# oval-group/GNN_branching

Measured on AMD Instinct MI355X. Metric: ReLU branching scores/sec (subproblems x ambiguous-ReLUs/s), higher is better.
Workload: dtype f32 (bf16x3-split 64x64 blocks); 1 GPU; cifar_base_kw, 256 synthetic subproblems per rank x 1 rank(s) = 256, T=2, p=64, shipped cifar_trained_gnn weights; batch_per_rank=256, ranks=1, global_batch=256, parallelism=dp1

## Files before the change

### gnn_branching_amd/_lib.py

```python
import ctypes as C
import os
import subprocess
import sys

CSRC = os.path.join(os.path.dirname(os.path.abspath(__file__)), "csrc")
LIB_PATH = os.environ.get("GNNB_LIB", os.path.join(CSRC, "libgnnb.so"))
SOURCES = ["gnnb.hip", "gnnb_dev.h", "gnnb_k_mlp.h", "gnnb_k_gather.h", "gnnb_k_fusedq.h", "gnnb_k_edges.h", "gnnb_k_misc.h", "gnnb_pack.h", "gnnb_train.h", "gnnb_k_kw.h"]
HIPCC_FLAGS = ["--offload-arch=gfx950", "-O3", "-std=c++17", "-shared", "-fPIC", "-pthread"]

GNNB_CONV, GNNB_LINEAR, GNNB_RELU, GNNB_FLATTEN = 0, 1, 2, 3


class LayerDesc(C.Structure):
    _fields_ = [("kind", C.c_int32), ("c_in", C.c_int32), ("c_out", C.c_int32), ("kh", C.c_int32),
                ("kw", C.c_int32), ("stride", C.c_int32), ("pad", C.c_int32), ("n_in", C.c_int32),
                ("n_out", C.c_int32), ("weight", C.c_void_p), ("bias", C.c_void_p)]


class Batch(C.Structure):
    _fields_ = [("lb", C.POINTER(C.c_void_p)), ("ub", C.POINTER(C.c_void_p)),
                ("dual", C.POINTER(C.c_void_p)), ("primal", C.POINTER(C.c_void_p)),
                ("x_lp", C.c_void_p), ("prop_w", C.c_void_p), ("prop_b", C.c_void_p), ("mask", C.c_void_p),
                ("n_graph", C.c_int32), ("n_relu", C.c_int32), ("n_primal", C.c_int32)]

# ... 20 lines not shown
    ("gnnb_get_option", C.c_int, [C.c_void_p, C.c_char_p, C.POINTER(C.c_int)]),
    ("gnnb_option_count", C.c_int, []),
    ("gnnb_option_name", C.c_char_p, [C.c_int]),
    ("gnnb_babsr", C.c_int, [C.c_void_p, C.POINTER(C.c_void_p), C.POINTER(C.c_void_p), C.c_int, C.c_void_p, C.c_void_p,
                             C.c_int, C.c_void_p, C.c_void_p, C.c_void_p]),
    ("gnnb_kw_workspace_bytes", C.c_size_t, [C.c_void_p, C.c_int]),
    ("gnnb_kw_bounds", C.c_int, [C.c_void_p, C.POINTER(KwBatch), C.c_int, C.POINTER(C.c_void_p), C.POINTER(C.c_void_p), C.POINTER(C.c_void_p),
                                 C.POINTER(C.c_void_p), C.c_void_p, C.c_void_p, C.c_size_t, C.c_void_p]),
    ("gnnb_mu_projection", C.c_int, [C.c_void_p, C.c_int, C.POINTER(C.c_int)]),
    ("gnnb_destroy", C.c_int, [C.c_void_p]),
    ("gnnb_get_weights", C.c_int, [C.c_void_p, C.c_void_p, C.c_size_t]),
    ("gnnb_set_weights", C.c_int, [C.c_void_p, C.c_void_p, C.c_size_t]),
    ("gnnb_online_create", C.c_int, [C.c_void_p, C.c_float, C.c_float]),
    ("gnnb_online_step", C.c_int, [C.c_void_p, C.POINTER(Batch), C.c_int, C.c_void_p, C.c_void_p, C.c_void_p, C.c_void_p,
                                   C.c_int, C.c_void_p]),
    ("gnnb_online_grad", C.c_int, [C.c_void_p, C.c_void_p, C.c_size_t]),
    ("gnnb_last_error", C.c_char_p, []),
    ("gnnb_abi_version", C.c_int, []),
    ("gnnb_build_id", C.c_char_p, []),
    ("gnnb_describe", C.c_int, [C.c_void_p, C.c_char_p, C.c_size_t]),
    ("gnnb_mu_location", C.c_int, [C.c_void_p, C.c_int, C.c_int, C.POINTER(C.c_size_t), C.POINTER(C.c_size_t)]),
    ("gnnb_set_halfpass_limit", C.c_int, [C.c_void_p, C.c_int]),
    ("gnnb_debug_occupy", C.c_int, [C.c_int, C.c_int, C.c_size_t, C.c_double, C.c_void_p]),
    ("gnnb_profile_enable", C.c_int, [C.c_void_p, C.c_int]),
    ("gnnb_profile_classes", C.c_int, []),
    ("gnnb_profile_class_name", C.c_char_p, [C.c_int]),
    ("gnnb_profile_read", C.c_int, [C.c_void_p, C.POINTER(C.c_double), C.POINTER(C.c_int64), C.c_int, C.c_int]),
    ("gnnb_profile_trace", C.c_int, [C.c_void_p, C.POINTER(C.c_int), C.POINTER(C.c_double), C.c_int]),
]


OPTION_ENV = {
    "GNNB_BF3": ("bf3", lambda v: int(v != 0)),
    "GNNB_FUSE": ("fuse", lambda v: int(v != 0)),
    "GNNB_NO_TOP": ("top", lambda v: int(v == 0)),
    "GNNB_NO_GATHER": ("gather", lambda v: int(v == 0)),
    "GNNB_NO_EMBED_FUSE": ("embed_fuse", lambda v: int(v == 0)),
    "GNNB_NO_DENSE_LDS": ("dense_lds", lambda v: int(v == 0)),
    "GNNB_TAIL_MAX_B": ("tail_max_b", lambda v: max(0, min(v, 1 << 30))),
    "GNNB_TOP_SPLIT": ("top_split", lambda v: 4 if v >= 4 else (2 if v >= 2 else 1)),
    "GNNB_TOP_FUSE_UPD": ("top_fuse_upd", lambda v: int(v != 0)),
    "GNNB_CLSPRE_MAX_B": ("clspre_max_b", lambda v: max(0, min(v, 1 << 30))),
}
OPTIONS = tuple(sorted({o for o, _ in OPTION_ENV.values()}))


# ... 99 lines not shown
```

### gnn_branching_amd/csrc/gnnb.hip

```cpp
#include <hip/hip_runtime.h>

#include <cmath>
#include <cstdarg>
#include <cstdio>
#include <cstdlib>
#include <cstring>
#include <string>
#include <vector>
#include <thread>
#include <unistd.h>
#include <sched.h>
#include <atomic>
#include <condition_variable>
#include <functional>
#include <mutex>

#include "../../include/gnnb.h"
#include "gnnb_pack.h"
#include "gnnb_train.h"

using namespace gnnb;

typedef float f32x16 __attribute__((ext_vector_type(16)));
typedef float f32x4 __attribute__((ext_vector_type(4)));
// ... 261 lines not shown
}

extern "C" int gnnb_create(gnnb_t** out, const float* w_blob, size_t n_floats, int T, int p) {
  if (!out || !w_blob) return fail(GNNB_E_INVALID, "gnnb_create: null argument");
  if (p != P) return fail(GNNB_E_INVALID, "gnnb_create: embedding size %d unsupported (kernels are built for p=64)", p);
  if (T < 1 || T > 16) return fail(GNNB_E_INVALID, "gnnb_create: T=%d out of range", T);
  if (n_floats != blob_floats()) return fail(GNNB_E_INVALID, "gnnb_create: weight blob has %zu floats, expected %zu", n_floats, blob_floats());
  int ndev = 0;
  hipError_t e = hipGetDeviceCount(&ndev);
  if (e != hipSuccess || ndev == 0) return fail(GNNB_E_HIP, "gnnb_create: no HIP device (%s)", hipGetErrorString(e));
  gnnb_t* h = new gnnb_handle();
  h->T = T;
  h->p = p;
  HIPCHK(hipGetDevice(&h->device));
  hipDeviceProp_t prop;
  HIPCHK(hipGetDeviceProperties(&prop, h->device));
  h->n_cu = prop.multiProcessorCount > 0 ? prop.multiProcessorCount : 256;
  if (int rc = load_weights(h, w_blob, nullptr)) return rc;
  HIPCHK(hipMalloc((void**)&h->d_zero, 256 * sizeof(float)));
  HIPCHK(hipMemset(h->d_zero, 0, 256 * sizeof(float)));
  HIPCHK(hipMalloc((void**)&h->d_ctl, 8 * 64 * sizeof(int)));
  HIPCHK(hipMemset(h->d_ctl, 0, 8 * 64 * sizeof(int)));
  HIPCHK(hipFuncSetAttribute((const void*)k_pre<false>, hipFuncAttributeMaxDynamicSharedMemorySize, (PackPreFwd::FLOATS + PackPreBwd::FLOATS) * 4));
  HIPCHK(hipFuncSetAttribute((const void*)k_pre<true>, hipFuncAttributeMaxDynamicSharedMemorySize, PackPreBwdL3::FLOATS * 4));
  HIPCHK(hipFuncSetAttribute((const void*)k_pre_inp, hipFuncAttributeMaxDynamicSharedMemorySize, PackPreInp::FLOATS * 4));
  HIPCHK(hipFuncSetAttribute((const void*)k_node_update<8, false>, hipFuncAttributeMaxDynamicSharedMemorySize, (PackUpd::FLOATS + 4096) * 4));
  HIPCHK(hipFuncSetAttribute((const void*)k_node_update<8, true>, hipFuncAttributeMaxDynamicSharedMemorySize, (PackUpd::FLOATS + 4096) * 4));
  HIPCHK(hipFuncSetAttribute((const void*)k_node_update<8, false, true>, hipFuncAttributeMaxDynamicSharedMemorySize, (PackUpd::FLOATS + 4096) * 4));
  HIPCHK(hipFuncSetAttribute((const void*)k_node_update<8, true, true>, hipFuncAttributeMaxDynamicSharedMemorySize, (PackUpd::FLOATS + 4096) * 4));
  HIPCHK(hipFuncSetAttribute((const void*)k_node_update<12, false, false, true>, hipFuncAttributeMaxDynamicSharedMemorySize, (PackUpdL3::FLOATS + 6144) * 4));
  HIPCHK(hipFuncSetAttribute((const void*)k_node_update<12, true, false, true>, hipFuncAttributeMaxDynamicSharedMemorySize, (PackUpdL3::FLOATS + 6144) * 4));
  HIPCHK(hipFuncSetAttribute((const void*)k_node_update<12, false, true, true>, hipFuncAttributeMaxDynamicSharedMemorySize, (PackUpdL3::FLOATS + 6144) * 4));
  HIPCHK(hipFuncSetAttribute((const void*)k_node_update<12, true, true, true>, hipFuncAttributeMaxDynamicSharedMemorySize, (PackUpdL3::FLOATS + 6144) * 4));
  HIPCHK(hipFuncSetAttribute((const void*)k_input_update, hipFuncAttributeMaxDynamicSharedMemorySize, PackUpdInp::FLOATS * 4));
  HIPCHK(hipFuncSetAttribute((const void*)k_score, hipFuncAttributeMaxDynamicSharedMemorySize, PackScore::FLOATS * 4));
  HIPCHK(hipFuncSetAttribute((const void*)k_gather<false>, hipFuncAttributeMaxDynamicSharedMemorySize, 128 * 1024));
  HIPCHK(hipFuncSetAttribute((const void*)k_gather<true>, hipFuncAttributeMaxDynamicSharedMemorySize, 128 * 1024));
  HIPCHK(hipFuncSetAttribute((const void*)k_gather16<false>, hipFuncAttributeMaxDynamicSharedMemorySize, 128 * 1024));
  HIPCHK(hipFuncSetAttribute((const void*)k_gather16<true>, hipFuncAttributeMaxDynamicSharedMemorySize, 128 * 1024));
  HIPCHK(hipFuncSetAttribute((const void*)k_gather16<false, true>, hipFuncAttributeMaxDynamicSharedMemorySize, 128 * 1024));
  HIPCHK(hipFuncSetAttribute((const void*)k_livesum, hipFuncAttributeMaxDynamicSharedMemorySize, 160 * 1024));
  HIPCHK(hipFuncSetAttribute((const void*)k_gather_input_update<true, false>, hipFuncAttributeMaxDynamicSharedMemorySize, 160 * 1024));
  HIPCHK(hipFuncSetAttribute((const void*)k_gather_input_update<true, true>, hipFuncAttributeMaxDynamicSharedMemorySize, 160 * 1024));
  HIPCHK(hipFuncSetAttribute((const void*)k_gather<false, true>, hipFuncAttributeMaxDynamicSharedMemorySize, 128 * 1024));

#define FUSEDQ_ATTR(L, S, P) HIPCHK(hipFuncSetAttribute((const void*)k_gather_update_q<L, S, P>, hipFuncAttributeMaxDynamicSharedMemorySize, 160 * 1024))
  FUSEDQ_ATTR(16, 0, false); FUSEDQ_ATTR(16, 1, false); FUSEDQ_ATTR(16, 2, false); FUSEDQ_ATTR(32, 1, false); FUSEDQ_ATTR(32, 1, true);
// ... 471 lines not shown

extern "C" int gnnb_mu_location(const gnnb_t* h, int B, int k, size_t* offset_bytes, size_t* n_floats) {
  if (!h || !h->bound) return fail(GNNB_E_STATE, "gnnb_mu_location: no network bound");
  if (k < 0 || k >= (int)h->N.size() || B < 1) return fail(GNNB_E_INVALID, "gnnb_mu_location: bad layer/batch");
  WsLayout w = ws_layout(h, B);
  if (offset_bytes) *offset_bytes = w.mu[k] * sizeof(float);
  if (n_floats) *n_floats = (size_t)B * h->N[k] * 64;
  return GNNB_OK;
}

extern "C" int gnnb_mu_projection(const gnnb_t* h, int k, int* linear_id) {
  if (!h || !linear_id) return fail(GNNB_E_INVALID, "gnnb_mu_projection: null argument");
  if (k < 0 || k >= (int)h->N.size()) return fail(GNNB_E_INVALID, "gnnb_mu_projection: bad layer");
  *linear_id = k < MAXL + 2 ? h->last_proj[k] : -1;
  return GNNB_OK;
}

extern "C" int gnnb_set_halfpass_limit(gnnb_t* h, int n) {
  if (!h) return fail(GNNB_E_INVALID, "null handle");
  h->halfpass_limit = n;
  return GNNB_OK;
}

extern "C" int gnnb_debug_occupy(int n_workgroups, int threads, size_t lds_bytes, double ms, void* stream) {
  if (n_workgroups < 1 || n_workgroups > 4096 || threads < 64 || threads > 1024 || lds_bytes > 160 * 1024 || !(ms > 0.0) || ms > 500.0)
    return fail(GNNB_E_INVALID, "gnnb_debug_occupy: bad arguments");
  static bool attr = false;
  if (!attr) { HIPCHK(hipFuncSetAttribute((const void*)k_occupy, hipFuncAttributeMaxDynamicSharedMemorySize, 160 * 1024)); attr = true; }
  hipLaunchKernelGGL(k_occupy, dim3((unsigned)n_workgroups), dim3((unsigned)threads), lds_bytes, (hipStream_t)stream, (unsigned long long)(ms * 1e5));
  hipError_t e = hipGetLastError();
  if (e != hipSuccess) return fail(GNNB_E_HIP, "launch of k_occupy failed: %s", hipGetErrorString(e));
  return GNNB_OK;
}

extern "C" int gnnb_profile_enable(gnnb_t* h, int on) {
  if (!h) return fail(GNNB_E_INVALID, "null handle");
  h->prof = on != 0;
  return GNNB_OK;
}
extern "C" int gnnb_profile_classes(void) { return PC_COUNT; }
extern "C" const char* gnnb_profile_class_name(int cls) { return (cls >= 0 && cls < PC_COUNT) ? kProfNames[cls] : ""; }
extern "C" int gnnb_profile_read(gnnb_t* h, double* total_ms, int64_t* launches, int n, int reset) {
  if (!h) return fail(GNNB_E_INVALID, "null handle");
  if (!h->pending.empty()) {
    for (auto& ev : h->pending) {
      HIPCHK(hipEventSynchronize(ev.b));
// ... 176 lines not shown
    a.njobs = q;
    if (q == 0) return;
    int maxn = 0;
    for (int k = 0; k <= L; ++k) maxn = std::max(maxn, h->N[k]);
    a.lv_floats = (maxn + 3) & ~3;
    if ((size_t)(a.lv_floats + maxw) * 4 > 160 * 1024) {
      for (int i = 0; i < q; ++i) a.job[i].wlds = 0;
      maxw = 0;
    }
    lz.run(PC_LIVESUM, [&] { hipLaunchKernelGGL(k_livesum, dim3((unsigned)B, (unsigned)q), dim3(256), (size_t)(a.lv_floats + maxw) * sizeof(float), st, a); });
  }
  void input_embedding() {
    const long G = (long)B * h->N[0];
    EmbedArgs a{h->d_pack[PK_EMBED] + PackEmbed::W, h->d_pack[PK_EMBED] + PackEmbed::B, in->lb[0], in->x_lp, in->ub[0], mu(0), G};
    long grid = (G + 16 * EMBED_UNROLL - 1) / (16 * EMBED_UNROLL);
    if (grid > (long)h->n_cu * 16) grid = (long)h->n_cu * 16;
    if (!p.embed_in_gather) lz.run(PC_EMBED, [&] { hipLaunchKernelGGL(k_embed, dim3((unsigned)grid), dim3(256), 0, st, a); });
    proj[0] = L_INP_F_1;
  }
  void pre() {
    long nt = 0;
    for (int k = 1; k <= L; ++k) nt += (((long)B * h->N[k] + 31) / 32) * 2;
    const PreAllArgs a = pre_args();
    const size_t lds = (h->bf3 ? (size_t)PackPreBwdL3::FLOATS : (size_t)PackPreFwd::FLOATS + PackPreBwd::FLOATS) * 4;
    void (*kern)(PreAllArgs) = h->bf3 ? k_pre<true> : k_pre<false>;
    lz.run(PC_PRE, [&] { hipLaunchKernelGGL(kern, dim3(mlp_grid(h, nt / 8)), dim3(PRE_WAVES * 64), lds, st, a); });
  }
  void pre_inp() {
    const long G = (long)B * h->N[0];
    const TileMap tm = bwd_map(h, 0);
    const long nt = map_tiles(tm, B);
    PreArgs a{h->d_pack[PK_PRE_INP], in->lb[0], in->ub[0], nullptr, nullptr, nullptr, nullptr, ws + w.Q, G, nt, h->N[0], 1,
              to_dtm(tm), nullptr, nullptr};
    lz.run(PC_PRE_INP, [&] { hipLaunchKernelGGL(k_pre_inp, dim3(mlp_grid(h, nt)), dim3(WG_MLP), PackPreInp::FLOATS * 4, st, a); });
  }

  bool embed_src(int k) const { return k == 1 && p.embed_in_gather && proj[0] == L_INP_F_1; }
  GArgs gather_args(const DevGather& d, int k, const float* src, bool scored, bool sparse, int src_layer, float* sout) const {
    return GArgs{in->lb[k], in->ub[k], in->mask, src, nb, map_tiles(d.g.tm, B), scored ? 1 : 0, h->R, roff[k], to_dtm(d.g.tm), to_dg(d, h->d_zero),
                 EmbedSrc{in->lb[0], in->x_lp, in->ub[0], h->d_pack[PK_EMBED]}, sparse ? in->lb[src_layer] : nullptr,
                 sparse ? in->ub[src_layer] : nullptr, sparse ? sout : nullptr};
  }
  void gather(const DevGather& d, int k, const float* src, bool scored, bool embed, int src_layer, float* sout) {
    const bool sparse = !embed && src_layer >= 1;
    const GArgs a = gather_args(d, k, src, scored, sparse, src_layer, sout);
    const size_t lds = gather_lds_bytes(d, 0) + (sparse ? sparse_tab_bytes(d) : 0) + (d.g.lanes == 16 ? 16 + (size_t)WAVES_MLP * STAGE16_FLOATS * 4 : 0);
    constexpr int kGatherOcc = 2;
// ... 866 lines not shown
```

### gnn_branching_amd/csrc/gnnb_dev.h

```cpp
#pragma once

struct Frag {
  f32x16 t[2];
};

#define FRAG_AT(x, R) ((x).t[(R) >> 4][(R)&15])

__device__ __forceinline__ f32x16 mfma32(float a, float b, f32x16 c) {
  return __builtin_amdgcn_mfma_f32_32x32x2f32(a, b, c, 0, 0, 0);
}

template <int KSTEPS, class GetB>
__device__ __forceinline__ void gemm_w64(const float* wl, int lane, Frag& acc, GetB getB) {
  const f32x4* w4 = reinterpret_cast<const f32x4*>(wl) + lane;
  f32x4 a0 = w4[0], a1 = w4[64];
#pragma unroll
  for (int s4 = 0; s4 < KSTEPS / 4; ++s4) {
    f32x4 n0 = a0, n1 = a1;
    if (s4 + 1 < KSTEPS / 4) {
      n0 = w4[((s4 + 1) * 2 + 0) * 64];
      n1 = w4[((s4 + 1) * 2 + 1) * 64];
    }
    __builtin_amdgcn_sched_barrier(0);
#pragma unroll
// ... 28 lines not shown

__device__ __forceinline__ void split_pair_bf3(float a, float b, unsigned& u1, unsigned& u2, unsigned& u3);
template <class GetB>
__device__ __forceinline__ void split_bf3(GetB& getB, int fk, u32x4& p1, u32x4& p2, u32x4& p3) {
#pragma unroll
  for (int q = 0; q < 4; ++q) {
    unsigned u1, u2, u3;
    split_pair_bf3(getB(8 * fk + 2 * q), getB(8 * fk + 2 * q + 1), u1, u2, u3);
    p1[q] = u1; p2[q] = u2; p3[q] = u3;
  }
}

__device__ __forceinline__ void split_pair_bf3(float a, float b, unsigned& u1, unsigned& u2, unsigned& u3) {
  u1 = pk_bf16(a, b);
  const float ra = a - __uint_as_float(u1 << 16), rb = b - __uint_as_float(u1 & 0xffff0000u);
  u2 = pk_bf16(ra, rb);
  const float sa = ra - __uint_as_float(u2 << 16), sb = rb - __uint_as_float(u2 & 0xffff0000u);
  u3 = pk_bf16(sa, sb);
}

#ifndef GEMM_BF3_PIPE
#define GEMM_BF3_PIPE 1
#endif
template <int NFRAG, bool PIPE = (GEMM_BF3_PIPE != 0), class GetB>
__device__ __forceinline__ void gemm_w64_bf3(const float* wl, int lane, Frag& acc, GetB getB) {
  const u32x4* w = reinterpret_cast<const u32x4*>(wl) + lane;
  if constexpr (PIPE) {
  u32x4 p1, p2, p3;
  split_bf3(getB, 0, p1, p2, p3);
  __builtin_amdgcn_sched_barrier(0);
#pragma unroll
  for (int fk = 0; fk < 4 * NFRAG; ++fk) {
    const bf16x8 x1 = __builtin_bit_cast(bf16x8, p1), x2 = __builtin_bit_cast(bf16x8, p2), x3 = __builtin_bit_cast(bf16x8, p3);
    const bf16x8 w1a = __builtin_bit_cast(bf16x8, w[((fk * 2 + 0) * 3 + 0) * 64]), w1b = __builtin_bit_cast(bf16x8, w[((fk * 2 + 1) * 3 + 0) * 64]);
    const bf16x8 w2a = __builtin_bit_cast(bf16x8, w[((fk * 2 + 0) * 3 + 1) * 64]), w2b = __builtin_bit_cast(bf16x8, w[((fk * 2 + 1) * 3 + 1) * 64]);
    const bf16x8 w3a = __builtin_bit_cast(bf16x8, w[((fk * 2 + 0) * 3 + 2) * 64]), w3b = __builtin_bit_cast(bf16x8, w[((fk * 2 + 1) * 3 + 2) * 64]);
    acc.t[0] = mfma_bf16(w3a, x1, acc.t[0]);
    acc.t[1] = mfma_bf16(w3b, x1, acc.t[1]);
    acc.t[0] = mfma_bf16(w2a, x2, acc.t[0]);
    acc.t[1] = mfma_bf16(w2b, x2, acc.t[1]);
    acc.t[0] = mfma_bf16(w1a, x3, acc.t[0]);
    acc.t[1] = mfma_bf16(w1b, x3, acc.t[1]);
    acc.t[0] = mfma_bf16(w2a, x1, acc.t[0]);
    acc.t[1] = mfma_bf16(w2b, x1, acc.t[1]);
    acc.t[0] = mfma_bf16(w1a, x2, acc.t[0]);
    acc.t[1] = mfma_bf16(w1b, x2, acc.t[1]);
    acc.t[0] = mfma_bf16(w1a, x1, acc.t[0]);
    acc.t[1] = mfma_bf16(w1b, x1, acc.t[1]);
    if (fk + 1 < 4 * NFRAG) split_bf3(getB, fk + 1, p1, p2, p3);
// ... 139 lines not shown
      const int i = i0 + u * stride;
      if (i < n4) l[i] = v[u];
    }
  }
}
__device__ __forceinline__ void copy_to_lds_part(float* lds, const float* src, int nfloats, int tid, int nthr) {
  const f32x4* g = reinterpret_cast<const f32x4*>(src);
  f32x4* l = reinterpret_cast<f32x4*>(lds);
  const int n4 = nfloats / 4;
  for (int i0 = tid; i0 < n4; i0 += 8 * nthr) {
    f32x4 v[8];
#pragma unroll
    for (int u = 0; u < 8; ++u) {
      const int i = i0 + u * nthr;
      v[u] = g[i < n4 ? i : i0];
    }
#pragma unroll
    for (int u = 0; u < 8; ++u) {
      const int i = i0 + u * nthr;
      if (i < n4) l[i] = v[u];
    }
  }
}

__device__ __forceinline__ void stage_pack(float* lds, const float* pack, int nfloats) {
  copy_to_lds(lds, pack, nfloats);
  __syncthreads();
}

struct DTileMap { int mode, N, C, H, W, CT, PY, PX, ay, ax, NBY, NBX, NCG, TPS, lpy, lpx; unsigned tps_magic; };
__device__ __forceinline__ int tile_sample(const DTileMap& tm, long tile) {
  const unsigned n = (unsigned)__builtin_amdgcn_readfirstlane((int)tile), d = (unsigned)tm.TPS;
  if (d <= 1u) return (int)n;
  unsigned q = __umulhi(n, tm.tps_magic);
  if (q * d > n) --q;
  return (int)q;
}
struct TileCtx { long sample; int n, cg, by, bx, y, x; bool valid; };

__device__ __forceinline__ TileCtx tile_decode(const DTileMap& tm, long tile, int j, long total_rows) {
  TileCtx c;
  if (tm.mode == 0) {
    const long g = tile * 32 + j;
    c.valid = g < total_rows;
    const long gc = c.valid ? g : total_rows - 1;
    c.sample = gc / tm.N;
// ... 64 lines not shown
```

### gnn_branching_amd/csrc/gnnb_k_misc.h

```cpp
#pragma once

struct LiveSumJob {
  int kind;
  const float* w;
  const float* lf;
  float* out;
  int Ndst, Nsrc, ld, normalise;
  int c_in, h_in, w_in, c_out, h_out, w_out, kh, kw, stride, pad;
  int wlds;
};
struct LiveSumArgs { int njobs, B, lv_floats; LiveSumJob job[2 * MAXL]; };
#define LIVESUM_MAXW 16384

#define LIVESUM_MAXSRC 40000
#define LS_CC 4
#define LS_DO 9
template <int KH, int KW, int S, bool FWD, int NT>
__device__ __forceinline__ void livesum_conv(const LiveSumJob& jb, const float* lv, const float* W, float* out, int tid) {
  const int kh = KH ? KH : jb.kh, kw = KH ? KW : jb.kw, st = KH ? S : jb.stride;
  const int Hd = FWD ? jb.h_out : jb.h_in, Wd = FWD ? jb.w_out : jb.w_in, Cd = FWD ? jb.c_out : jb.c_in;
  const int Hs = FWD ? jb.h_in : jb.h_out, Ws = FWD ? jb.w_in : jb.w_out, Cs = FWD ? jb.c_in : jb.c_out;
  const int npos = Hd * Wd;
  const int P = npos < NT ? npos : NT;
  const int ngrp = NT / P;
// ... 582 lines not shown
    if (i < nrec) {
      const int* r = a.image + 16 + i * AMBREC_WORDS;
      const int k = r[0], g = r[1];
      if ((unsigned)k >= (unsigned)a.L || g < 0 || (long)g >= a.G[k]) {
        if (a.status) atomicOr(a.status, 4);
        continue;
      }
      a.dual[k][(long)g * 3 + 1] = __int_as_float(r[2]);
      a.dual[k][(long)g * 3 + 2] = __int_as_float(r[3]);
      a.z_pre[k][g] = __int_as_float(r[4]);
      a.z_post[k][g] = __int_as_float(r[5]);
    } else {
      a.z_out[i - nrec] = __int_as_float(a.image[16 + nrec * AMBREC_WORDS + (i - nrec)]);
    }
  }
}

__global__ void k_occupy(unsigned long long ticks) {
  extern __shared__ __attribute__((aligned(16))) float lds[];
  if (threadIdx.x == 0) lds[0] = 0.0f;
  const unsigned long long t0 = __builtin_amdgcn_s_memrealtime();
  while (__builtin_amdgcn_s_memrealtime() - t0 < ticks) __builtin_amdgcn_s_sleep(64);
}
```

### gnn_branching_amd/csrc/gnnb_k_mlp.h

```cpp
#pragma once

struct EmbedArgs { const float* w; const float* b; const float* lb; const float* x; const float* ub; float* mu; long G; };

#define EMBED_UNROLL 4
__global__ __launch_bounds__(256) void k_embed(EmbedArgs a) {
  const int q = threadIdx.x & 15;
  float w[4][3], bias[4];
#pragma unroll
  for (int c = 0; c < 4; ++c) {
    bias[c] = a.b[4 * q + c];
#pragma unroll
    for (int i = 0; i < 3; ++i) w[c][i] = a.w[(4 * q + c) * 3 + i];
  }
  const long nodes_per_pass = (long)gridDim.x * 16;
  long g = (long)blockIdx.x * 16 + (threadIdx.x >> 4);
  for (; g < a.G; g += nodes_per_pass * EMBED_UNROLL) {
    float l[EMBED_UNROLL], x[EMBED_UNROLL], u[EMBED_UNROLL];
#pragma unroll
    for (int r = 0; r < EMBED_UNROLL; ++r) {
      const long gg = g + r * nodes_per_pass;
      const long gc = gg < a.G ? gg : a.G - 1;
      l[r] = a.lb[gc]; x[r] = a.x[gc]; u[r] = a.ub[gc];
    }
#pragma unroll
// ... 119 lines not shown
  float* P;
  long G, ntiles;
  int N, hw;
  DTileMap tm;
  const int* list;
  const int* cnt;
};

struct PreAllArgs {
  const float* pack_f;
  const float* pack_b;
  int L, do_bwd;
  const float* lb[MAXL]; const float* ub[MAXL]; const float* dual[MAXL];
  const float* z_pre[MAXL]; const float* z_post[MAXL]; const float* bias[MAXL];
  float* Pf[MAXL]; float* Pb[MAXL];
  const int* list[MAXL];
  const int* cnt;
  int N[MAXL], hw[MAXL];
};

#ifndef PRE_PIPE
#define PRE_PIPE false
#endif
template <bool BF3>
__device__ __forceinline__ void pre_tile(const PreAllArgs& a, const float* lds, const float* lds_b, int k, bool bwd, const int* list, int count,
                                         long t, int lane) {
  constexpr int F_W1 = BF3 ? (int)PackPreFwdL3::W1 : (int)PackPreFwd::W1, F_B1 = BF3 ? (int)PackPreFwdL3::B1 : (int)PackPreFwd::B1;
  constexpr int F_B2 = BF3 ? (int)PackPreFwdL3::B2 : (int)PackPreFwd::B2;
  constexpr int B_W1 = BF3 ? (int)PackPreBwdL3::W1 : (int)PackPreBwd::W1, B_B1 = BF3 ? (int)PackPreBwdL3::B1 : (int)PackPreBwd::B1;
  constexpr int B_B2 = BF3 ? (int)PackPreBwdL3::B2 : (int)PackPreBwd::B2, B_B3 = BF3 ? (int)PackPreBwdL3::B3 : (int)PackPreBwd::B3;
  constexpr int B_W4 = (int)PackPreBwd::W4, B_B4 = BF3 ? (int)PackPreBwdL3::B4 : (int)PackPreBwd::B4;
  constexpr int B_B5 = BF3 ? (int)PackPreBwdL3::B5 : (int)PackPreBwd::B5;
  const int h = lane >> 5, j = lane & 31;
  {
    const long idx = t * 32 + j;
    const bool valid = idx < count;
    const long gc = list[valid ? idx : 0];
    const int n = (int)(gc % a.N[k]);
    const float lb = a.lb[k][gc], ub = a.ub[k][gc];
    const Ratio r = compute_ratio(lb, ub);
    const float d1 = a.dual[k][gc * 3 + 1], d2 = a.dual[k][gc * 3 + 2];
    const float c = a.bias[k][n / a.hw[k]];
    const float zpre = a.z_pre[k][gc], zpost = a.z_post[k][gc];
    float x[4];
    if (!bwd) {
      x[0] = h ? lb : r.beta;
      x[1] = h ? (d1 - d2) : ub;
      x[2] = h ? zpost : zpre;
      x[3] = h ? 0.0f : c;
      Frag H;
      frag_bias(H, lds + F_B1, h);
      gemm_small<4>(lds + F_W1, lane, H, x);
      frag_relu(H);
      Frag Pf;
      frag_bias(Pf, lds + F_B2, h);
      if (BF3) gemm_w64_bf3<1, PRE_PIPE>(lds + PackPreFwdL3::W23, lane, Pf, [&](int s) { return FRAG_AT(H, s); });
      else gemm_w64<32>(lds + PackPreFwd::W2, lane, Pf, [&](int s) { return FRAG_AT(H, s); });
      if (valid) frag_store_rows(Pf, a.Pf[k], gc, h);
    } else {
      x[0] = h ? ub : lb;
      x[1] = h ? (-d2 + d1) : r.beta;
      x[2] = h ? zpre : zpost;
      x[3] = h ? 0.0f : c;
      Frag H1;
      frag_bias(H1, lds_b + B_B1, h);
      gemm_small<4>(lds_b + B_W1, lane, H1, x);
      frag_relu(H1);
      Frag H2;
      frag_bias(H2, lds_b + B_B2, h);
      if (BF3) gemm_w64_bf3<1, PRE_PIPE>(lds_b + PackPreBwdL3::W23, lane, H2, [&](int s) { return FRAG_AT(H1, s); });
      else gemm_w64<32>(lds_b + PackPreBwd::W2, lane, H2, [&](int s) { return FRAG_AT(H1, s); });
      frag_relu(H2);
      Frag S;
      frag_bias(S, lds_b + B_B3, h);
      if (BF3) gemm_w64_bf3<1, PRE_PIPE>(lds_b + PackPreBwdL3::W33, lane, S, [&](int s) { return FRAG_AT(H2, s); });
      else gemm_w64<32>(lds_b + PackPreBwd::W3, lane, S, [&](int s) { return FRAG_AT(H2, s); });
      const float nd2 = -d2;
      Frag H4;
      frag_bias(H4, lds_b + B_B4, h);
      auto in4 = [&](int s) {
        const float v = FRAG_AT(S, s & 31);
        return s < 32 ? v : (s < 64 ? v * nd2 : v * d1);
      };
      if (BF3) gemm_w64_bf3<3, PRE_PIPE>(lds_b + PackPreBwdL3::W43, lane, H4, in4);
      else gemm_w64<96>(lds_b + B_W4, lane, H4, in4);
      frag_relu(H4);
      Frag Pb;
      frag_bias(Pb, lds_b + B_B5, h);
      if (BF3) gemm_w64_bf3<1, PRE_PIPE>(lds_b + PackPreBwdL3::W53, lane, Pb, [&](int s) { return FRAG_AT(H4, s); });
      else gemm_w64<32>(lds_b + PackPreBwd::W5, lane, Pb, [&](int s) { return FRAG_AT(H4, s); });
      if (valid) frag_store_rows(Pb, a.Pb[k], gc, h);
    }
  }
}

#ifndef PRE_WAVES
#define PRE_WAVES 16
#endif
template <bool BF3>
__global__ __launch_bounds__(PRE_WAVES * 64) void k_pre(PreAllArgs a) {
  extern __shared__ __attribute__((aligned(16))) float lds[];
  const int lane = threadIdx.x & 63, wave = threadIdx.x >> 6;
  long nhalf = 0;
  for (int k = 0; k < a.L; ++k) nhalf += (long)((a.cnt[4 * k + 1] + 31) / 32);
  auto run = [&](long t, bool bwd, const float* lf, const float* lb) {
    int k = 0, count = 0;
    for (; k < a.L; ++k) {
      count = a.cnt[4 * k + 1];
      const long tk = (count + 31) / 32;
      if (t < tk) break;
      t -= tk;
    }
    pre_tile<BF3>(a, lf, lb, k, bwd, a.list[k], count, t, lane);
  };
  if (BF3) {
    copy_to_lds(lds + PackPreFwdL3::W1, a.pack_f + PackPreFwd::W1, 512 + 64);
    copy_to_lds(lds + PackPreFwdL3::B2, a.pack_f + PackPreFwd::B2, 64);
    copy_to_lds(lds + PackPreFwdL3::W23, a.pack_f + PackPreFwd::W23, 6144);
    if (a.do_bwd) {
      copy_to_lds(lds + PackPreBwdL3::B3, a.pack_b + PackPreBwd::B3, 64);
      copy_to_lds(lds + PackPreBwdL3::B4, a.pack_b + PackPreBwd::B4, 64);
      copy_to_lds(lds + PackPreBwdL3::B5, a.pack_b + PackPreBwd::B5, 64);
      copy_to_lds(lds + PackPreBwdL3::W33, a.pack_b + PackPreBwd::W33, 6144);
      copy_to_lds(lds + PackPreBwdL3::W43, a.pack_b + PackPreBwd::W43, 18432);
      copy_to_lds(lds + PackPreBwdL3::W53, a.pack_b + PackPreBwd::W53, 6144);
    }
    __syncthreads();
    for (long t = (long)wave * gridDim.x + blockIdx.x; t < nhalf; t += (long)gridDim.x * PRE_WAVES) run(t, false, lds, lds);
    if (!a.do_bwd) return;
    __syncthreads();
    copy_to_lds(lds + PackPreBwdL3::W1, a.pack_b + PackPreBwd::W1, 512 + 64);
    copy_to_lds(lds + PackPreBwdL3::B2, a.pack_b + PackPreBwd::B2, 64);
    copy_to_lds(lds + PackPreBwdL3::W23, a.pack_b + PackPreBwd::W23, 6144);
    __syncthreads();
    for (long t = (long)wave * gridDim.x + blockIdx.x; t < nhalf; t += (long)gridDim.x * PRE_WAVES) run(t, true, lds, lds);
    return;
  }
  float* lds_b = lds + (int)PackPreFwd::FLOATS;
  copy_to_lds(lds_b, a.pack_b, PackPreBwd::FLOATS);
  stage_pack(lds, a.pack_f, PackPreFwd::FLOATS);
  const long ntiles = nhalf * (a.do_bwd ? 2 : 1);
  for (long tile = (long)wave * gridDim.x + blockIdx.x; tile < ntiles; tile += (long)gridDim.x * PRE_WAVES) {
    const bool bwd = a.do_bwd && tile < nhalf;
    run((a.do_bwd && !bwd) ? tile - nhalf : tile, bwd, lds, lds_b);
  }
}

static_assert(CLS_THREADS == PRE_WAVES * 64, "k_classify_pre: one block = the 16 waves of k_pre");
#define CLSPRE_LDS_BYTES ((size_t)(PackPreBwdL3::FLOATS + CLS_BLOCK) * 4)
static_assert(CLSPRE_LDS_BYTES + 2048 <= 160 * 1024, "k_classify_pre: image + list + the classification's static LDS must fit one CU");
__global__ __launch_bounds__(CLS_THREADS) void k_classify_pre(ClassifyArgs ca, PreAllArgs a) {
  extern __shared__ __attribute__((aligned(16))) float lds[];
  int* amb_local = reinterpret_cast<int*>(lds + PackPreBwdL3::FLOATS);
  const int lane = threadIdx.x & 63, wave = threadIdx.x >> 6;
  copy_to_lds(lds + PackPreFwdL3::W1, a.pack_f + PackPreFwd::W1, 512 + 64);
  copy_to_lds(lds + PackPreFwdL3::B2, a.pack_f + PackPreFwd::B2, 64);
  copy_to_lds(lds + PackPreFwdL3::W23, a.pack_f + PackPreFwd::W23, 6144);
  if (a.do_bwd) {
    copy_to_lds(lds + PackPreBwdL3::B3, a.pack_b + PackPreBwd::B3, 64);
    copy_to_lds(lds + PackPreBwdL3::B4, a.pack_b + PackPreBwd::B4, 64);
// ... 191 lines not shown
```

### include/gnnb.h

```cpp
#ifndef GNNB_H
#define GNNB_H

#include <stddef.h>
#include <stdint.h>

#ifdef __cplusplus
extern "C" {
#endif

#define GNNB_ABI_VERSION 2

enum {
  GNNB_OK = 0,
  GNNB_E_INVALID = -1,
  GNNB_E_HIP = -2,
  GNNB_E_STATE = -3,
  GNNB_E_NOMEM = -4
};

enum { GNNB_CONV = 0, GNNB_LINEAR = 1, GNNB_RELU = 2, GNNB_FLATTEN = 3 };

typedef struct gnnb_handle gnnb_t;

typedef struct {
// ... 66 lines not shown

int gnnb_online_create(gnnb_t* h, float lr, float weight_decay);

int gnnb_online_step(gnnb_t* h, const gnnb_batch* in, int B, const int32_t* kw_index, const float* improvement,
                     float* loss, float* scores_padded, int apply, void* stream);

int gnnb_online_grad(const gnnb_t* h, float* grad, size_t n_floats);

const char* gnnb_last_error(void);
int gnnb_abi_version(void);
const char* gnnb_build_id(void);


int gnnb_describe(const gnnb_t* h, char* buf, size_t cap);

int gnnb_mu_location(const gnnb_t* h, int B, int k, size_t* offset_bytes, size_t* n_floats);

int gnnb_mu_projection(const gnnb_t* h, int k, int* linear_id);

int gnnb_set_halfpass_limit(gnnb_t* h, int n);

int gnnb_debug_occupy(int n_workgroups, int threads, size_t lds_bytes, double ms, void* stream);

int gnnb_profile_enable(gnnb_t* h, int on);
int gnnb_profile_classes(void);
const char* gnnb_profile_class_name(int cls);
int gnnb_profile_read(gnnb_t* h, double* total_ms, int64_t* launches, int n, int reset);
int gnnb_profile_trace(gnnb_t* h, int* cls, double* ms, int cap);

#ifdef __cplusplus
}
#endif
#endif
```

Baseline: 77.00 million scores/s.

## Stage bf3 pre-kernel weights via async LDS DMA in one pass with prefetch

In the bf3 path, k_pre now loads its weights into LDS with global_load_lds DMA, spread across the waves. The forward W23 weights are no longer staged; they are read straight from global memory through buffer loads. This removes the old two-phase structure, which needed a second staging pass and an extra barrier between the forward and backward tiles. All tiles now run from one unified loop, and each tile's inputs are prefetched before the DMA wait so the loads overlap the staging. The cost is that the forward GEMM reads its weights from global or L2 instead of LDS, and a debug entry point is added to check the staged image.

After: 77.64 million scores/s, median of 6. Within noise of the previous version (+0.8%).

```diff
diff --git a/gnn_branching_amd/_lib.py b/gnn_branching_amd/_lib.py
--- a/gnn_branching_amd/_lib.py
+++ b/gnn_branching_amd/_lib.py
@@ -66,6 +66,7 @@
     ("gnnb_mu_location", C.c_int, [C.c_void_p, C.c_int, C.c_int, C.POINTER(C.c_size_t), C.POINTER(C.c_size_t)]),
     ("gnnb_set_halfpass_limit", C.c_int, [C.c_void_p, C.c_int]),
     ("gnnb_debug_occupy", C.c_int, [C.c_int, C.c_int, C.c_size_t, C.c_double, C.c_void_p]),
+    ("gnnb_debug_stage_image", C.c_int, [C.c_void_p, C.c_int, C.c_int, C.c_int, C.c_void_p, C.c_void_p, C.c_size_t, C.POINTER(C.c_size_t)]),
     ("gnnb_profile_enable", C.c_int, [C.c_void_p, C.c_int]),
     ("gnnb_profile_classes", C.c_int, []),
     ("gnnb_profile_class_name", C.c_char_p, [C.c_int]),
diff --git a/gnn_branching_amd/csrc/gnnb.hip b/gnn_branching_amd/csrc/gnnb.hip
--- a/gnn_branching_amd/csrc/gnnb.hip
+++ b/gnn_branching_amd/csrc/gnnb.hip
@@ -307,7 +307,7 @@
   HIPCHK(hipMalloc((void**)&h->d_ctl, 8 * 64 * sizeof(int)));
   HIPCHK(hipMemset(h->d_ctl, 0, 8 * 64 * sizeof(int)));
   HIPCHK(hipFuncSetAttribute((const void*)k_pre<false>, hipFuncAttributeMaxDynamicSharedMemorySize, (PackPreFwd::FLOATS + PackPreBwd::FLOATS) * 4));
-  HIPCHK(hipFuncSetAttribute((const void*)k_pre<true>, hipFuncAttributeMaxDynamicSharedMemorySize, PackPreBwdL3::FLOATS * 4));
+  HIPCHK(hipFuncSetAttribute((const void*)k_pre<true>, hipFuncAttributeMaxDynamicSharedMemorySize, PRE1_FLOATS * 4));
   HIPCHK(hipFuncSetAttribute((const void*)k_pre_inp, hipFuncAttributeMaxDynamicSharedMemorySize, PackPreInp::FLOATS * 4));
   HIPCHK(hipFuncSetAttribute((const void*)k_node_update<8, false>, hipFuncAttributeMaxDynamicSharedMemorySize, (PackUpd::FLOATS + 4096) * 4));
   HIPCHK(hipFuncSetAttribute((const void*)k_node_update<8, true>, hipFuncAttributeMaxDynamicSharedMemorySize, (PackUpd::FLOATS + 4096) * 4));
@@ -825,6 +825,44 @@
   return GNNB_OK;
 }
 
+extern "C" int gnnb_debug_stage_image(gnnb_t* h, int kind, int first_thread, int n_threads, float* lds_out, float* want, size_t cap_floats,
+                                      size_t* image_floats) {
+  if (!h || !h->bound || !h->d_pack[0]) return fail(GNNB_E_STATE, "gnnb_debug_stage_image: no network bound / no weights");
+  if (kind < 0 || kind >= IMG_KINDS || !lds_out || !want || !image_floats) return fail(GNNB_E_INVALID, "gnnb_debug_stage_image: bad arguments");
+  if (first_thread != 0 || n_threads != PRE_WAVES * 64) return fail(GNNB_E_INVALID, "gnnb_debug_stage_image: image %d is staged by a whole workgroup of %d threads", kind, PRE_WAVES * 64);
+  const int lead = 64;
+  std::vector<float> img(PRE1_FLOATS);
+  auto put = [&](size_t at, const std::vector<float>& src, size_t from, size_t n) { std::memcpy(img.data() + at, src.data() + from, n * sizeof(float)); };
+  const Packs& pk = h->packs;
+  put(PackPreBwdL3::W1, pk.pre_bwd, PackPreBwd::W1, 512 + 64);
+  put(PackPreBwdL3::B2, pk.pre_bwd, PackPreBwd::B2, 64);
+  put(PackPreBwdL3::W23, pk.pre_bwd, PackPreBwd::W23, 6144);
+  put(PackPreBwdL3::B3, pk.pre_bwd, PackPreBwd::B3, 64);
+  put(PackPreBwdL3::B4, pk.pre_bwd, PackPreBwd::B4, 64);
+  put(PackPreBwdL3::B5, pk.pre_bwd, PackPreBwd::B5, 64);
+  put(PackPreBwdL3::W33, pk.pre_bwd, PackPreBwd::W33, 6144);
+  put(PackPreBwdL3::W43, pk.pre_bwd, PackPreBwd::W43, 18432);
+  put(PackPreBwdL3::W53, pk.pre_bwd, PackPreBwd::W53, 6144);
+  put(PRE1_FWD + PackPreFwdL3::W1, pk.pre_fwd, PackPreFwd::W1, 512 + 64);
+  put(PRE1_FWD + PackPreFwdL3::B2, pk.pre_fwd, PackPreFwd::B2, 64);
+  const size_t total = img.size() + 2 * lead;
+  *image_floats = img.size();
+  if (total > cap_floats || total * 4 > 160 * 1024) return fail(GNNB_E_INVALID, "gnnb_debug_stage_image: %zu floats needed", total);
+  float* d_out = nullptr;
+  HIPCHK(hipMalloc((void**)&d_out, total * 4));
+  const StageImgArgs a{kind, lead, (int)total, h->d_pack[PK_PRE_FWD], h->d_pack[PK_PRE_BWD], d_out};
+  static bool attr = false;
+  if (!attr) { HIPCHK(hipFuncSetAttribute((const void*)k_debug_stage, hipFuncAttributeMaxDynamicSharedMemorySize, 160 * 1024)); attr = true; }
+  hipLaunchKernelGGL(k_debug_stage, dim3(1), dim3((unsigned)n_threads), total * 4, (hipStream_t)0, a);
+  hipError_t e = hipGetLastError();
+  if (e == hipSuccess) e = hipMemcpy(lds_out, d_out, total * 4, hipMemcpyDeviceToHost);
+  (void)hipFree(d_out);
+  if (e != hipSuccess) return fail(GNNB_E_HIP, "k_debug_stage failed: %s", hipGetErrorString(e));
+  for (size_t i = 0; i < total; ++i) want[i] = __builtin_bit_cast(float, STAGE_CANARY);
+  std::memcpy(want + lead, img.data(), img.size() * 4);
+  return GNNB_OK;
+}
+
 extern "C" int gnnb_debug_occupy(int n_workgroups, int threads, size_t lds_bytes, double ms, void* stream) {
   if (n_workgroups < 1 || n_workgroups > 4096 || threads < 64 || threads > 1024 || lds_bytes > 160 * 1024 || !(ms > 0.0) || ms > 500.0)
     return fail(GNNB_E_INVALID, "gnnb_debug_occupy: bad arguments");
@@ -1047,7 +1085,7 @@
     long nt = 0;
     for (int k = 1; k <= L; ++k) nt += (((long)B * h->N[k] + 31) / 32) * 2;
     const PreAllArgs a = pre_args();
-    const size_t lds = (h->bf3 ? (size_t)PackPreBwdL3::FLOATS : (size_t)PackPreFwd::FLOATS + PackPreBwd::FLOATS) * 4;
+    const size_t lds = (h->bf3 ? (size_t)PRE1_FLOATS : (size_t)PackPreFwd::FLOATS + PackPreBwd::FLOATS) * 4;
     void (*kern)(PreAllArgs) = h->bf3 ? k_pre<true> : k_pre<false>;
     lz.run(PC_PRE, [&] { hipLaunchKernelGGL(kern, dim3(mlp_grid(h, nt / 8)), dim3(PRE_WAVES * 64), lds, st, a); });
   }
diff --git a/gnn_branching_amd/csrc/gnnb_dev.h b/gnn_branching_amd/csrc/gnnb_dev.h
--- a/gnn_branching_amd/csrc/gnnb_dev.h
+++ b/gnn_branching_amd/csrc/gnnb_dev.h
@@ -74,9 +74,17 @@
 #ifndef GEMM_BF3_PIPE
 #define GEMM_BF3_PIPE 1
 #endif
-template <int NFRAG, bool PIPE = (GEMM_BF3_PIPE != 0), class GetB>
+template <int NFRAG, bool PIPE = (GEMM_BF3_PIPE != 0), bool WGLOBAL = false, class GetB>
 __device__ __forceinline__ void gemm_w64_bf3(const float* wl, int lane, Frag& acc, GetB getB) {
-  const u32x4* w = reinterpret_cast<const u32x4*>(wl) + lane;
+  struct WImage {
+    const u32x4* l; __amdgpu_buffer_rsrc_t r; int vo;
+    __device__ __forceinline__ u32x4 operator[](int i) const {
+      if constexpr (WGLOBAL) return __builtin_amdgcn_raw_buffer_load_b128(r, vo, i * 16, 0);
+      else return l[i];
+    }
+  };
+  const WImage w{reinterpret_cast<const u32x4*>(wl) + (WGLOBAL ? 0 : lane),
+                 __builtin_amdgcn_make_buffer_rsrc(const_cast<float*>(wl), 0, WGLOBAL ? NFRAG * 6144 * 4 : 0, 0x00020000), lane * 16};
   if constexpr (PIPE) {
   u32x4 p1, p2, p3;
   split_bf3(getB, 0, p1, p2, p3);
@@ -262,6 +270,16 @@
     }
   }
 }
+
+__device__ __forceinline__ void stage_dma(float* lds_dst, const float* gsrc, int nfloats, int tid, int nthr) {
+  typedef __attribute__((address_space(3))) void lds_void;
+  typedef const __attribute__((address_space(1))) void glb_void;
+  const int n4 = nfloats >> 2, lane = tid & 63;
+  const int first = __builtin_amdgcn_readfirstlane(tid >> 6) * 64, step = (nthr >> 6) * 64;
+  for (int c = first; c < n4; c += step)
+    if (c + lane < n4) __builtin_amdgcn_global_load_lds((glb_void*)(gsrc + 4 * (c + lane)), (lds_void*)(lds_dst + 4 * c), 16, 0, 0);
+}
+__device__ __forceinline__ void stage_dma_wait() { asm volatile("s_waitcnt vmcnt(0)" ::: "memory"); }
 
 __device__ __forceinline__ void stage_pack(float* lds, const float* pack, int nfloats) {
   copy_to_lds(lds, pack, nfloats);
diff --git a/gnn_branching_amd/csrc/gnnb_k_misc.h b/gnn_branching_amd/csrc/gnnb_k_misc.h
--- a/gnn_branching_amd/csrc/gnnb_k_misc.h
+++ b/gnn_branching_amd/csrc/gnnb_k_misc.h
@@ -628,3 +628,16 @@
   const unsigned long long t0 = __builtin_amdgcn_s_memrealtime();
   while (__builtin_amdgcn_s_memrealtime() - t0 < ticks) __builtin_amdgcn_s_sleep(64);
 }
+
+#define STAGE_CANARY 0xcacacacau
+enum { IMG_PRE = 0, IMG_KINDS = 1 };
+struct StageImgArgs { int kind, lead, total; const float *p0, *p1; float* out; };
+__global__ __launch_bounds__(1024) void k_debug_stage(StageImgArgs a) {
+  extern __shared__ __attribute__((aligned(16))) float lds[];
+  for (int i = threadIdx.x; i < a.total; i += blockDim.x) lds[i] = __uint_as_float(STAGE_CANARY);
+  __syncthreads();
+  if (a.kind == IMG_PRE) stage_pre_image(lds + a.lead, a.p0, a.p1, true, threadIdx.x);
+  stage_dma_wait();
+  __syncthreads();
+  for (int i = threadIdx.x; i < a.total; i += blockDim.x) a.out[i] = lds[i];
+}
diff --git a/gnn_branching_amd/csrc/gnnb_k_mlp.h b/gnn_branching_amd/csrc/gnnb_k_mlp.h
--- a/gnn_branching_amd/csrc/gnnb_k_mlp.h
+++ b/gnn_branching_amd/csrc/gnnb_k_mlp.h
@@ -165,26 +165,37 @@
 #ifndef PRE_PIPE
 #define PRE_PIPE false
 #endif
-template <bool BF3>
-__device__ __forceinline__ void pre_tile(const PreAllArgs& a, const float* lds, const float* lds_b, int k, bool bwd, const int* list, int count,
-                                         long t, int lane) {
+struct PreIn { long gc; bool valid; float lb, ub, d1, d2, c, zpre, zpost; };
+__device__ __forceinline__ PreIn pre_fetch(const PreAllArgs& a, int k, const int* list, int count, long t, int lane) {
+  PreIn in;
+  const long idx = t * 32 + (lane & 31);
+  in.valid = idx < count;
+  in.gc = list[in.valid ? idx : 0];
+  const int n = (int)(in.gc % a.N[k]);
+  in.lb = a.lb[k][in.gc]; in.ub = a.ub[k][in.gc];
+  in.d1 = a.dual[k][in.gc * 3 + 1]; in.d2 = a.dual[k][in.gc * 3 + 2];
+  in.c = a.bias[k][n / a.hw[k]];
+  in.zpre = a.z_pre[k][in.gc]; in.zpost = a.z_post[k][in.gc];
+  return in;
+}
+template <bool BF3, bool W23F_GLOBAL = false>
+__device__ __forceinline__ void pre_chain(const PreAllArgs& a, const float* lds, const float* lds_b, const float* w23f, int k, bool bwd,
+                                          const PreIn& in, int lane) {
   constexpr int F_W1 = BF3 ? (int)PackPreFwdL3::W1 : (int)PackPreFwd::W1, F_B1 = BF3 ? (int)PackPreFwdL3::B1 : (int)PackPreFwd::B1;
   constexpr int F_B2 = BF3 ? (int)PackPreFwdL3::B2 : (int)PackPreFwd::B2;
   constexpr int B_W1 = BF3 ? (int)PackPreBwdL3::W1 : (int)PackPreBwd::W1, B_B1 = BF3 ? (int)PackPreBwdL3::B1 : (int)PackPreBwd::B1;
   constexpr int B_B2 = BF3 ? (int)PackPreBwdL3::B2 : (int)PackPreBwd::B2, B_B3 = BF3 ? (int)PackPreBwdL3::B3 : (int)PackPreBwd::B3;
   constexpr int B_W4 = (int)PackPreBwd::W4, B_B4 = BF3 ? (int)PackPreBwdL3::B4 : (int)PackPreBwd::B4;
   constexpr int B_B5 = BF3 ? (int)PackPreBwdL3::B5 : (int)PackPreBwd::B5;
-  const int h = lane >> 5, j = lane & 31;
+  const int h = lane >> 5;
   {
-    const long idx = t * 32 + j;
-    const bool valid = idx < count;
-    const long gc = list[valid ? idx : 0];
-    const int n = (int)(gc % a.N[k]);
-    const float lb = a.lb[k][gc], ub = a.ub[k][gc];
+    const long gc = in.gc;
+    const bool valid = in.valid;
+    const float lb = in.lb, ub = in.ub;
     const Ratio r = compute_ratio(lb, ub);
-    const float d1 = a.dual[k][gc * 3 + 1], d2 = a.dual[k][gc * 3 + 2];
-    const float c = a.bias[k][n / a.hw[k]];
-    const float zpre = a.z_pre[k][gc], zpost = a.z_post[k][gc];
+    const float d1 = in.d1, d2 = in.d2;
+    const float c = in.c;
+    const float zpre = in.zpre, zpost = in.zpost;
     float x[4];
     if (!bwd) {
       x[0] = h ? lb : r.beta;
@@ -197,7 +208,8 @@
       frag_relu(H);
       Frag Pf;
       frag_bias(Pf, lds + F_B2, h);
-      if (BF3) gemm_w64_bf3<1, PRE_PIPE>(lds + PackPreFwdL3::W23, lane, Pf, [&](int s) { return FRAG_AT(H, s); });
+      if (BF3 && W23F_GLOBAL) gemm_w64_bf3<1, PRE_PIPE, true>(w23f, lane, Pf, [&](int s) { return FRAG_AT(H, s); });
+      else if (BF3) gemm_w64_bf3<1, PRE_PIPE>(w23f, lane, Pf, [&](int s) { return FRAG_AT(H, s); });
       else gemm_w64<32>(lds + PackPreFwd::W2, lane, Pf, [&](int s) { return FRAG_AT(H, s); });
       if (valid) frag_store_rows(Pf, a.Pf[k], gc, h);
     } else {
@@ -236,14 +248,77 @@
     }
   }
 }
+template <bool BF3>
+__device__ __forceinline__ void pre_tile(const PreAllArgs& a, const float* lds, const float* lds_b, int k, bool bwd, const int* list, int count,
+                                         long t, int lane) {
+  pre_chain<BF3>(a, lds, lds_b, lds + PackPreFwdL3::W23, k, bwd, pre_fetch(a, k, list, count, t, lane), lane);
+}
 
 #ifndef PRE_WAVES
 #define PRE_WAVES 16
 #endif
+#define PRE1_FWD ((int)PackPreBwdL3::FLOATS)
+#define PRE1_FLOATS (PRE1_FWD + (int)PackPreFwdL3::W23)
+static_assert((size_t)PRE1_FLOATS * 4 <= 160 * 1024, "k_pre: the backward image and the forward small pieces must fit one CU");
+__device__ __forceinline__ void stage_pre_image(float* lds, const float* pack_f, const float* pack_b, bool do_bwd, int tid) {
+  constexpr int NT = PRE_WAVES * 64;
+  auto rot = [&](int w) { return (tid + 64 * w) & (NT - 1); };
+  float* lf = lds + PRE1_FWD;
+  stage_dma(lf + PackPreFwdL3::W1, pack_f + PackPreFwd::W1, 512 + 64, rot(1), NT);
+  stage_dma(lf + PackPreFwdL3::B2, pack_f + PackPreFwd::B2, 64, rot(2), NT);
+  if (!do_bwd) return;
+  stage_dma(lds + PackPreBwdL3::W1, pack_b + PackPreBwd::W1, 512 + 64, rot(3), NT);
+  stage_dma(lds + PackPreBwdL3::B2, pack_b + PackPreBwd::B2, 64, rot(4), NT);
+  stage_dma(lds + PackPreBwdL3::B3, pack_b + PackPreBwd::B3, 64, rot(5), NT);
+  stage_dma(lds + PackPreBwdL3::B4, pack_b + PackPreBwd::B4, 64, rot(6), NT);
+  stage_dma(lds + PackPreBwdL3::B5, pack_b + PackPreBwd::B5, 64, rot(7), NT);
+  stage_dma(lds + PackPreBwdL3::W23, pack_b + PackPreBwd::W23, 6144, tid, NT);
+  stage_dma(lds + PackPreBwdL3::W33, pack_b + PackPreBwd::W33, 6144, rot(8), NT);
+  stage_dma(lds + PackPreBwdL3::W53, pack_b + PackPreBwd::W53, 6144, tid, NT);
+  stage_dma(lds + PackPreBwdL3::W43, pack_b + PackPreBwd::W43, 18432, rot(8), NT);
+}
+
 template <bool BF3>
 __global__ __launch_bounds__(PRE_WAVES * 64) void k_pre(PreAllArgs a) {
   extern __shared__ __attribute__((aligned(16))) float lds[];
   const int lane = threadIdx.x & 63, wave = threadIdx.x >> 6;
+  if (BF3) {
+    stage_pre_image(lds, a.pack_f, a.pack_b, a.do_bwd != 0, threadIdx.x);
+    long nhalf = 0;
+    for (int k = 0; k < a.L; ++k) nhalf += (long)((a.cnt[4 * k + 1] + 31) / 32);
+    const long ntiles = nhalf * (a.do_bwd ? 2 : 1);
+    const float* lds_f = lds + PRE1_FWD;
+    const float* w23f = a.pack_f + PackPreFwd::W23;
+    auto locate = [&](long tile, bool& bwd, int& k, int& count, long& t) {
+      bwd = a.do_bwd && tile < nhalf;
+      t = (a.do_bwd && !bwd) ? tile - nhalf : tile;
+      for (k = 0; k < a.L; ++k) {
+        count = a.cnt[4 * k + 1];
+        const long tk = (count + 31) / 32;
+        if (t < tk) break;
+        t -= tk;
+      }
+    };
+    long tile = (long)__builtin_amdgcn_readfirstlane(wave) * gridDim.x + blockIdx.x;
+    bool bwd = false;
+    int k = 0, count = 0;
+    long t = 0;
+    PreIn in{};
+    if (tile < ntiles) {
+      locate(tile, bwd, k, count, t);
+      in = pre_fetch(a, k, a.list[k], count, t, lane);
+    }
+    stage_dma_wait();
+    __syncthreads();
+    for (; tile < ntiles;) {
+      pre_chain<true, true>(a, lds_f, lds, w23f, k, bwd, in, lane);
+      tile += (long)gridDim.x * PRE_WAVES;
+      if (tile >= ntiles) break;
+      locate(tile, bwd, k, count, t);
+      in = pre_fetch(a, k, a.list[k], count, t, lane);
+    }
+    return;
+  }
   long nhalf = 0;
   for (int k = 0; k < a.L; ++k) nhalf += (long)((a.cnt[4 * k + 1] + 31) / 32);
   auto run = [&](long t, bool bwd, const float* lf, const float* lb) {
@@ -256,29 +331,6 @@
     }
     pre_tile<BF3>(a, lf, lb, k, bwd, a.list[k], count, t, lane);
   };
-  if (BF3) {
-    copy_to_lds(lds + PackPreFwdL3::W1, a.pack_f + PackPreFwd::W1, 512 + 64);
-    copy_to_lds(lds + PackPreFwdL3::B2, a.pack_f + PackPreFwd::B2, 64);
-    copy_to_lds(lds + PackPreFwdL3::W23, a.pack_f + PackPreFwd::W23, 6144);
-    if (a.do_bwd) {
-      copy_to_lds(lds + PackPreBwdL3::B3, a.pack_b + PackPreBwd::B3, 64);
-      copy_to_lds(lds + PackPreBwdL3::B4, a.pack_b + PackPreBwd::B4, 64);
-      copy_to_lds(lds + PackPreBwdL3::B5, a.pack_b + PackPreBwd::B5, 64);
-      copy_to_lds(lds + PackPreBwdL3::W33, a.pack_b + PackPreBwd::W33, 6144);
-      copy_to_lds(lds + PackPreBwdL3::W43, a.pack_b + PackPreBwd::W43, 18432);
-      copy_to_lds(lds + PackPreBwdL3::W53, a.pack_b + PackPreBwd::W53, 6144);
-    }
-    __syncthreads();
-    for (long t = (long)wave * gridDim.x + blockIdx.x; t < nhalf; t += (long)gridDim.x * PRE_WAVES) run(t, false, lds, lds);
-    if (!a.do_bwd) return;
-    __syncthreads();
-    copy_to_lds(lds + PackPreBwdL3::W1, a.pack_b + PackPreBwd::W1, 512 + 64);
-    copy_to_lds(lds + PackPreBwdL3::B2, a.pack_b + PackPreBwd::B2, 64);
-    copy_to_lds(lds + PackPreBwdL3::W23, a.pack_b + PackPreBwd::W23, 6144);
-    __syncthreads();
-    for (long t = (long)wave * gridDim.x + blockIdx.x; t < nhalf; t += (long)gridDim.x * PRE_WAVES) run(t, true, lds, lds);
-    return;
-  }
   float* lds_b = lds + (int)PackPreFwd::FLOATS;
   copy_to_lds(lds_b, a.pack_b, PackPreBwd::FLOATS);
   stage_pack(lds, a.pack_f, PackPreFwd::FLOATS);
diff --git a/include/gnnb.h b/include/gnnb.h
--- a/include/gnnb.h
+++ b/include/gnnb.h
@@ -112,6 +112,9 @@
 
 int gnnb_debug_occupy(int n_workgroups, int threads, size_t lds_bytes, double ms, void* stream);
 
+int gnnb_debug_stage_image(gnnb_t* h, int kind, int first_thread, int n_threads, float* lds_out, float* want, size_t cap_floats,
+                           size_t* image_floats);
+
 int gnnb_profile_enable(gnnb_t* h, int on);
 int gnnb_profile_classes(void);
 const char* gnnb_profile_class_name(int cls);
```
